# lkotipal/dccrg

Measured on AMD Instinct MI355X. Metric: cell-updates/s (node) for 3D advection w/ halo exchange; % of HBM roofline, higher is better.
Workload: dtype f64

## Files before the change

dccrg_amd/_lib.py:

```python
from __future__ import annotations

import ctypes as C
import os
import re

HERE = os.path.dirname(os.path.abspath(__file__))
LIB_PATH = os.path.join(HERE, os.path.basename(os.environ.get("DCCRGX_LIB", "libdccrgx.so")))
HEADER = os.path.join(os.path.dirname(HERE), "include", "dccrgx.h")

_lib = None

EXCHANGE_FN = C.CFUNCTYPE(C.c_int, C.c_void_p, C.POINTER(C.c_void_p), C.POINTER(C.c_size_t), C.POINTER(C.c_void_p),
                          C.POINTER(C.c_size_t))

u64 = C.c_uint64
i64 = C.c_int64
i32 = C.c_int32
sz = C.c_size_t
vp = C.c_void_p
P = C.POINTER

_SIGS = {
    "dccrgx_last_error": (C.c_char_p, []),
    "dccrgx_abi_version": (C.c_int, []),
# ... 103 lines not shown
    "dccrgx_particles_accelerate": (C.c_int, [vp, C.c_int, C.c_int, C.c_int, C.c_int, C.c_double]),
    "dccrgx_particles_deposit_moments": (C.c_int, [vp, C.c_int, C.c_int, C.c_int, C.c_int, P(C.c_int), P(C.c_int),
                                                   C.c_int, C.c_int]),
    "dccrgx_particles_boris": (C.c_int, [vp, C.c_int, C.c_int, C.c_int, C.c_int, C.c_int, C.c_double]),
    "dccrgx_gradient": (C.c_int, [vp, C.c_int, P(C.c_int), C.c_double, C.c_int]),
    "dccrgx_curl": (C.c_int, [vp, P(C.c_int), P(C.c_int), C.c_double, C.c_int, C.c_int]),
    "dccrgx_divergence": (C.c_int, [vp, P(C.c_int), C.c_int, C.c_double, C.c_int, C.c_int]),
    "dccrgx_field_axpy": (C.c_int, [vp, C.c_int, C.c_double, C.c_int, C.c_int]),
    "dccrgx_set_send_single_cells": (C.c_int, [vp, C.c_int]),
    "dccrgx_get_send_single_cells": (C.c_int, [vp, P(C.c_int)]),
    "dccrgx_set_field_window": (C.c_int, [vp, C.c_int, sz, sz]),
    "dccrgx_field_device_ptr": (C.c_int, [vp, C.c_int, P(vp)]),
    "dccrgx_field_upload": (C.c_int, [vp, C.c_int, sz, sz, vp]),
    "dccrgx_field_download": (C.c_int, [vp, C.c_int, sz, sz, vp]),
    "dccrgx_update_copies_of_remote_neighbors": (C.c_int, [vp]),
    "dccrgx_start_remote_neighbor_copy_updates": (C.c_int, [vp]),
    "dccrgx_wait_remote_neighbor_copy_update_receives": (C.c_int, [vp]),
    "dccrgx_wait_remote_neighbor_copy_update_sends": (C.c_int, [vp]),
    "dccrgx_wait_remote_neighbor_copy_updates": (C.c_int, [vp]),
    "dccrgx_gol_step": (C.c_int, [vp, C.c_int, C.c_int]),
    "dccrgx_gol_commit": (C.c_int, [vp, C.c_int]),
    "dccrgx_gol_amr": (C.c_int, [vp, C.c_int, C.c_int, C.c_int, C.c_int]),
    "dccrgx_get_live_neighbors": (C.c_int, [vp, C.c_int, C.c_int]),
    "dccrgx_advection_step": (C.c_int, [vp, P(C.c_int), C.c_double, C.c_int]),
    "dccrgx_advection_commit": (C.c_int, [vp, C.c_int]),
    "dccrgx_advection_initialize": (C.c_int, [vp, P(C.c_int)]),
    "dccrgx_advection_max_time_step": (C.c_int, [vp, P(C.c_int), P(C.c_double)]),
    "dccrgx_advection_max_time_step_device": (C.c_int, [vp, P(C.c_int), vp]),
    "dccrgx_advection_check_adaptation": (C.c_int, [vp, C.c_int, C.c_double, C.c_double, C.c_double, vp]),
    "dccrgx_advection_adapt": (C.c_int, [vp, vp, vp]),
    "dccrgx_advection_refine_candidates": (C.c_int, [vp, C.c_int, C.c_double, C.c_double, vp, sz, P(sz)]),
    "dccrgx_advection_layout": (C.c_int, [vp, P(u64)]),
    "dccrgx_advection_occupancy": (C.c_int, [vp, P(u64)]),
    "dccrgx_advection_length_source": (C.c_int, [vp, P(C.c_int), P(C.c_int)]),
    "dccrgx_poisson_cache": (C.c_int, [vp, C.c_int, C.c_int, vp, sz, vp, sz]),
    "dccrgx_poisson_solve": (C.c_int, [vp, C.c_uint, C.c_uint, C.c_double, C.c_double, C.c_double, C.c_int,
                                       P(C.c_uint), P(C.c_double)]),
    "dccrgx_poisson_field": (C.c_int, [vp, C.c_char_p, P(C.c_int)]),
    "dccrgx_allreduce_f64": (C.c_int, [vp, P(C.c_double), C.c_int, C.c_int]),
    "dccrgx_allreduce_f64_device": (C.c_int, [vp, vp, vp, C.c_int, C.c_int]),
    "dccrgx_barrier": (C.c_int, [vp]),
    "dccrgx_get_transport": (C.c_int, [vp, P(C.c_int), P(C.c_int)]),
    "dccrgx_comm_loopback": (C.c_int, [vp, C.c_int, sz, sz, sz]),
    "dccrgx_synchronize": (C.c_int, [vp]),
    "dccrgx_compute_stream": (vp, [vp]),
    "dccrgx_kernel_timing": (C.c_int, [vp, C.c_int, P(C.c_double), P(i64)]),
}


def header_symbols():
    with open(HEADER) as f:
        txt = f.read()
    return sorted(set(re.findall(r"\b(dccrgx_[a-z0-9_]+)\s*\(", txt)))


def lib():
    global _lib
    if _lib is not None:
        return _lib
    if not os.path.exists(LIB_PATH):
        raise ImportError(f"dccrg_amd native library missing: {LIB_PATH} (run python -m dccrg_amd.build)")
    L = C.CDLL(LIB_PATH)
    for name, (res, args) in _SIGS.items():
        fn = getattr(L, name)
        fn.restype = res
        fn.argtypes = args
# ... 18 lines not shown
```

dccrg_amd/csrc/api.hip:

```cpp
#include <algorithm>
#include <array>
#include <chrono>
#include <cmath>
#include <cstdio>
#include <cstring>
#include <limits>
#include <numeric>

#include <fcntl.h>
#include <unistd.h>

#include "dccrgx_grid.hpp"

namespace dccrgx {

static thread_local std::string g_last_error;

template <class F>
static int guard(F&& f) {
	try {
		return f();
	} catch (const Error& e) {
		g_last_error = e.what();
		return e.code;
// ... 2639 lines not shown
		const char* env = std::getenv("DCCRGX_NBREC");
		const bool rec_off = !(env && std::atoi(env) == 1);
		uint64_t per_ext = rec_off ? 40 : 32;
		const uint64_t n_irr_cells = n - out[9], ext_irr = g.total_ext - ext_reg;
		uint64_t own = 64, lvl_byte = 0;
		if (g.adv_fids_valid && ensure_len_table(g, g.adv_fids, false)) {
			per_ext = 16;
			lvl_byte = 1;
			if (DCCRGX_LEN_OWN) own = 40;
		}
		out[11] = own * n + (12 + (own == 40 ? lvl_byte : 0)) * n_irr_cells + (per_ext + lvl_byte + 4) * ext_irr +
		          per_ext * ext_reg + 8 * uint64_t(g.n_fine_faces) + 32 * nt;
		return 0;
	});
}

int dccrgx_advection_occupancy(dccrgx_grid* gp, uint64_t out[6]) {
	return guard([&] {
		GRID_OR_FAIL(gp);
		DX_REQUIRE(out, "null output");
		ensure_tiles(g);
		const bool valid = g.adv_fids_valid;
		const bool rec = valid && ensure_nbrec(g, g.adv_fids) != nullptr;
		const bool len = valid && ensure_len_table(g, g.adv_fids, false) != nullptr;
		for (int kind = 0; kind < 2; kind++) {
			const Grid::SweepLaunch& L = adv_sweep_launch(g, kind, rec, len);
			int k = 0;
			HIP_CHECK(hipOccupancyMaxActiveBlocksPerMultiprocessor(&k, L.fn, 512, L.lds));
			out[3 * kind] = uint64_t(L.blocks_per_cu);
			out[3 * kind + 1] = uint64_t(k);
			out[3 * kind + 2] = L.lds;
		}
		return 0;
	});
}

int dccrgx_advection_length_source(dccrgx_grid* gp, const int fids[7], int* out) {
	return guard([&] {
		GRID_OR_FAIL(gp);
		DX_REQUIRE(out, "null output");
		const double* f[7];
		adv_fields(g, fids, f);
		ensure_tiles(g);
		*out = ensure_len_table(g, fids, false) ? 1 : 0;
		return 0;
	});
}

int dccrgx_advection_commit(dccrgx_grid* gp, int df) {
	return guard([&] {
		GRID_OR_FAIL(gp);
		commit(g, field(g, df));
		g.adv_commits_on_mesh++;
		return 0;
	});
}

int dccrgx_advection_initialize(dccrgx_grid* gp, const int fids[7]) {
	return guard([&] {
		GRID_OR_FAIL(gp);
		const auto& ids = slot_ids_host(g);
		const size_t n = g.n_slots;
		for (int k = 0; k < 7; k++) g.adv_fids[k] = fids[k];
		g.adv_fids_valid = true;
		const bool stretched = g.str.active;
		for (int d = 0; d < 3 && stretched; d++)
// ... 544 lines not shown
```

dccrg_amd/csrc/dccrgx_internal.hpp:

```cpp
#pragma once

#include <hip/hip_runtime.h>
#include <rccl/rccl.h>

#include <atomic>
#include <cstdint>
#include <deque>
#include <map>
#include <stdexcept>
#include <string>
#include <unordered_map>
#include <unordered_set>
#include <vector>

#include "../../include/dccrgx.h"
#include "dccrgx_mapping.hpp"
#include "dccrgx_mesh.hpp"
#include "dccrgx_neighbors.hpp"

namespace dccrgx {

struct Error : std::runtime_error {
	int code;
	Error(int c, const std::string& s) : std::runtime_error(s), code(c) {}
// ... 705 lines not shown
                     size_t n_prefix = 0, const DevMesh* dm = nullptr, DBuf<int32_t>* src = nullptr,
                     const uint64_t* dS = nullptr, const uint64_t* dF = nullptr);

struct TileBuild {
	size_t n_tiles_inner = 0, n_tiles_outer = 0, max_ext = 0, total_ext = 0, n_fine = 0;
	std::vector<uint32_t> ext_off, ext_n, fine_off, fine_n;
};
TileBuild k_build_tiles(const uint32_t* face_ptr, const int32_t* face_ent, const uint64_t* slot_ids, const MapCtx& m,
                        bool morton, size_t n_inner, size_t n_local, int tile, DBuf<uint32_t>& tstart,
                        DBuf<uint32_t>& tell, DBuf<uint32_t>& ext_ptr, DBuf<uint32_t>& ext, DBuf<uint32_t>& ext_pk,
                        DBuf<uint32_t>& fine_base, DBuf<uint32_t>& tfine, hipStream_t s);

void k_classify_tiles(const MapCtx& m, const uint32_t* tstart, size_t n_tiles_inner, size_t n_tiles_outer,
                      const uint64_t* slot_ids, const int32_t* face_ell, DBuf<uint32_t>& lists, DBuf<int32_t>& tnb,
                      DBuf<RegTileMeta>& regmeta, size_t counts[4], hipStream_t s);

void k_pack(const uint8_t* field, size_t elem, size_t off, size_t len, const int32_t* slots, size_t n, uint8_t* out,
            hipStream_t s);
void k_place(const uint8_t* in, size_t elem, size_t off, size_t len, const int32_t* slots, size_t n, uint8_t* field,
             hipStream_t s);
void k_gol_csr(const uint32_t* state, uint32_t* out, const uint32_t* it_ptr, const int32_t* it_slot, size_t s0,
               size_t s1, hipStream_t s);
bool k_gol_structured(const uint32_t* state, uint32_t* out, const uint64_t n[3], const int per[3], const uint32_t* lo,
                      const uint32_t* hi, hipStream_t s);
void k_advection(const double* const f[7], double* rho_out, const uint32_t* face_ptr, const int32_t* face_ent,
                 size_t s0, size_t s1, double dt, hipStream_t s);
void k_advection_tiles(const double* const f[7], double* rho_out, Grid& g, int run, double dt, hipStream_t s,
                       const double* nbrec = nullptr, const double* lentab = nullptr);
const double* ensure_len_table(Grid& g, const int fids[7], bool sweep);
void k_len_check(const double* const f[7], const uint8_t* slot_lvl, size_t n, const double* tab, int* flag,
                 hipStream_t s);
void k_tile_levels(const uint8_t* slot_lvl, const uint32_t* ext_pk, size_t n_ext, uint8_t* ext_lvl,
                   RegTileMeta* regmeta, size_t n_reg, hipStream_t s);
#ifndef DCCRGX_LEN_OWN
#define DCCRGX_LEN_OWN 1
#endif
#ifndef DCCRGX_LEN_LDS
#define DCCRGX_LEN_LDS 0
#endif
#ifndef DCCRGX_LEN_LDS_GEN
#define DCCRGX_LEN_LDS_GEN DCCRGX_LEN_LDS
#endif
#ifndef DCCRGX_REG_BLOCKS
#define DCCRGX_REG_BLOCKS ((DCCRGX_LEN_OWN && !DCCRGX_LEN_LDS) ? 3 : 2)
#endif
#ifndef DCCRGX_GEN_BLOCKS
#define DCCRGX_GEN_BLOCKS ((DCCRGX_LEN_OWN && !DCCRGX_LEN_LDS_GEN) ? 3 : 2)
#endif
const Grid::SweepLaunch& adv_sweep_launch(Grid& g, int kind, bool nbrec, bool lentab);
const double* ensure_nbrec(Grid& g, const int fids[7]);
void k_nbrec(const double* const f[7], size_t n, double* r, hipStream_t s);
struct BandArgs {
	MapCtx m;
	const uint8_t* lvl8;
	const uint64_t* slot_ids;
	double inc, thr, uns;
	uint8_t* band;
};
void k_advection_ell(const double* const f[7], double* rho_out, const int32_t* ell, const int32_t* fine, size_t s0,
                     size_t s1, double dt, hipStream_t s, const BandArgs* bands = nullptr);
void k_adv_dt(const double* const f[7], size_t n, double* partial, size_t nblocks, hipStream_t s);
void k_min_partials(const double* partial, size_t n, double* out, hipStream_t s);
size_t k_adv_candidates(const MapCtx& m, const double* rho, const FaceView& F, const uint8_t* lvl8, size_t n,
                        double diff_increase, double diff_threshold, uint64_t* out, hipStream_t s);
struct AdvRequests {
	std::vector<uint64_t> refine, unrefine;
	DBuf<uint64_t> refine_dev;
	DBuf<uint64_t> unrefine_dev;
	size_t kept = 0;
	std::vector<size_t> part_slot;
	std::vector<uint32_t> part_len;
	std::vector<uint64_t> part_ids;
	std::vector<uint8_t> part_bands;
};
AdvRequests k_adv_requests(const MapCtx& m, const DevMesh& dm, const uint64_t* slot_ids, const uint8_t* band, size_t n,
                           bool solo, int rank, hipStream_t s);
void k_adv_bands(const MapCtx& m, const double* rho, const FaceView& F, const uint8_t* lvl8, size_t n,
                 double diff_increase, double diff_threshold, double unrefine_sensitivity, uint8_t* band,
                 hipStream_t s);
void k_adv_merge_parents(const MapCtx& m, const DevMesh& dm, size_t n_local, LazyIds& rm, double* rho,
// ... 65 lines not shown
```

dccrg_amd/csrc/mesh.hip:

```cpp
#include <algorithm>
#include <cstring>
#include <numeric>
#include <set>

#include "dccrgx_grid.hpp"

namespace dccrgx {

namespace {

__global__ void select_owner_kernel(const uint64_t* ids, const int32_t* own, size_t n, int rank, uint64_t* out,
                                    unsigned long long* counter) {
	const size_t i0 = (blockIdx.x * size_t(blockDim.x) + threadIdx.x) * kAppendRun;
	unsigned c = 0;
	for (int k = 0; k < kAppendRun; k++)
		if (i0 + k < n && own[i0 + k] == rank) c++;
	unsigned long long at = wave_reserve(counter, c);
	for (int k = 0; k < kAppendRun && c; k++)
		if (i0 + k < n && own[i0 + k] == rank) {
			out[at++] = ids[i0 + k];
			c--;
		}
}

// ... 688 lines not shown
	const auto ts = download(g.tstart.p, nt + 1, g.s_comp);
	const auto li = download(g.tlists.p + g.tcount[0] + g.tcount[1], ni, g.s_comp);
	std::vector<uint32_t> rec(8 * ni, 0u);
	bool fits = true;
	for (size_t i = 0; i < ni; i++) {
		const uint32_t t = li[i];
		uint32_t* r = &rec[8 * i];
		r[0] = ts[t];
		r[1] = ts[t + 1] - ts[t];
		r[2] = tb.ext_off[t];
		r[3] = tb.ext_n[t];
		r[4] = tb.fine_off[t];
		r[5] = tb.fine_n[t];
		if (r[3] > 1024u || r[5] > 512u || r[1] > 512u) fits = false;
	}
	if (std::getenv("DCCRGX_TILE_REASONS") && ni) {
		std::map<uint32_t, size_t> hist;
		uint32_t emax = 0;
		size_t etot = 0, ax_n[4] = {0, 0, 0, 0};
		const auto pk = download(g.ext_pk.p, g.total_ext, g.s_comp);
		for (size_t i = 0; i < ni; i++) {
			const uint32_t e = rec[8 * i + 3];
			hist[e / 128u * 128u]++;
			emax = std::max(emax, e);
			etot += e;
			for (uint32_t k = 0; k < e; k++) ax_n[__builtin_popcount(pk[rec[8 * i + 2] + k] >> 29)]++;
		}
		std::fprintf(stderr, "[tiles] irregular: %zu tiles, ext total %zu, max %u (all tiles: max %zu)\n", ni, etot, emax,
		             g.max_ext);
		for (auto& kv : hist) std::fprintf(stderr, "[tiles] ext %u..%u: %zu tiles\n", kv.first, kv.first + 127, kv.second);
		std::fprintf(stderr, "[tiles] ext axes per entry: 0:%zu 1:%zu 2:%zu 3:%zu\n", ax_n[0], ax_n[1], ax_n[2], ax_n[3]);
	}
	g.tmeta.release();
	if (fits && ni) upload(g.tmeta, rec, g.s_comp);
	g.tfused.release();
	g.tfused_n[0] = g.tfused_n[1] = 0;
#if DCCRGX_FUSED_SWEEP
	if (fits && nt) {
		const size_t nr = g.tcount[0] + g.tcount[1];
		const auto lr = download(g.tlists.p, nr, g.s_comp);
		std::vector<RegTileMeta> rm(nr);
		if (nr) d2h_small(rm.data(), g.tregmeta.p, nr * sizeof(RegTileMeta), g.s_comp);
		std::vector<int64_t> where(nt, -1);
		for (size_t i = 0; i < nr; i++) where[lr[i]] = int64_t(i);
		for (size_t i = 0; i < ni; i++) where[li[i]] = -int64_t(i) - 2;
		std::vector<uint32_t> fu(8 * nt, 0u);
		for (size_t t = 0; t < nt; t++) {
			uint32_t* r = &fu[8 * t];
			if (where[t] >= 0) {
				const RegTileMeta& m = rm[size_t(where[t])];
				r[0] = m.ts;
				for (int d = 0; d < 6; d++) r[1 + d] = uint32_t(m.nst[d]);
				r[7] = 1u;
			} else {
				const uint32_t* q = &rec[8 * size_t(-where[t] - 2)];
				for (int k = 0; k < 8; k++) r[k] = q[k];
			}
		}
		upload(g.tfused, fu, g.s_comp);
		g.tfused_n[0] = g.n_tiles_inner;
		g.tfused_n[1] = g.n_tiles_outer;
	}
#endif
	HIP_CHECK(hipStreamSynchronize(g.s_comp));
	DX_LAP("tiles.3_meta");
	g.tiles_valid = true;
	g.tiles_gen++;
// ... 80 lines not shown
```

dccrg_amd/csrc/sweep_kernels.hip:

```cpp
#include <cstring>
#include <cstdlib>

#include "dccrgx_internal.hpp"

namespace dccrgx {

namespace {

template <class T>
__global__ void pack_kernel(const T* __restrict__ f, const int32_t* __restrict__ slots, size_t n, T* __restrict__ out) {
	for (size_t i = blockIdx.x * size_t(blockDim.x) + threadIdx.x; i < n; i += size_t(gridDim.x) * blockDim.x)
		out[i] = f[slots[i]];
}

template <class T>
__global__ void place_kernel(const T* __restrict__ in, const int32_t* __restrict__ slots, size_t n, T* __restrict__ f) {
	for (size_t i = blockIdx.x * size_t(blockDim.x) + threadIdx.x; i < n; i += size_t(gridDim.x) * blockDim.x)
		f[slots[i]] = in[i];
}

__global__ void pack_bytes_kernel(const uint8_t* __restrict__ f, size_t elem, size_t off, size_t len,
                                  const int32_t* __restrict__ slots, size_t n, uint8_t* __restrict__ out) {
	for (size_t i = blockIdx.x * size_t(blockDim.x) + threadIdx.x; i < n * len; i += size_t(gridDim.x) * blockDim.x) {
		const size_t k = i / len, b = i - k * len;
// ... 905 lines not shown
	uint32_t tn = tk.next(t);
	uint32_t rec = tn < t1 ? tile_record_word(meta, tn, lane) : 0u;
	for (;;) {
		{
			RegSet ra;
			load(cur, ra);
			__syncthreads();
			stage(ra);
		}
		__syncthreads();
		const bool more = tn < t1;
		RM nxt = cur;
		if (more) {
			nxt = unpack(rec);
			const uint32_t tnn = tk.next(tn);
			rec = tnn < t1 ? tile_record_word(meta, tnn, lane) : 0u;
		}
		compute(cur);
		if (!more) break;
		cur = nxt;
		tn = tk.next(tn);
	}
}

struct TileMeta {
	uint32_t ts, n, e0, ne, fb, nf, pad0, pad1;
};

template <int MINW, bool REC, bool ONCE, bool LEN>
__global__ __launch_bounds__(512, MINW) void advection_tiles_pp_kernel(
    AdvPtrs P, double* __restrict__ rho_out, const uint32_t* __restrict__ tell, uint32_t tplane,
    const uint32_t* __restrict__ ext, const uint32_t* __restrict__ tfine, const TileMeta* __restrict__ meta,
    uint32_t ntiles, uint32_t ecap, double dt, const double* __restrict__ R, size_t nrec,
    const uint8_t* __restrict__ slvl, const uint8_t* __restrict__ extl, const double* __restrict__ LT) {
#pragma clang fp contract(off)
	static_assert(!(LEN && (REC || ONCE)), "the length table is for the default kernels only");
	constexpr bool LOWN = LEN && DCCRGX_LEN_OWN;
	constexpr bool LLVL = LOWN && !DCCRGX_LEN_LDS_GEN;
	constexpr uint32_t T = 512;
	constexpr uint32_t NROW = LLVL ? 4 : 7;
	extern __shared__ double shd[];
	const uint32_t W = T + ecap;
	double* shg = shd + NROW * W;
	uint32_t* shf = reinterpret_cast<uint32_t*>(shd + NROW * W + (ONCE ? 3 * T : 0));
	uint8_t* shok = reinterpret_cast<uint8_t*>(shf + 2 * T);
	double* lt = reinterpret_cast<double*>(shf + 2 * T);
	uint8_t* shl = reinterpret_cast<uint8_t*>(lt + 96);
	const StaticTiles tk(ntiles);
	const uint32_t t1 = tk.t1;
	uint32_t t = tk.first();
	if (t >= t1) return;
	const uint32_t tid = threadIdx.x;
	uint32_t ti = tid;
	const double* const rho = P.p[0];
	const double* const lx = P.p[1];
	const double* const ly = P.p[2];
	const double* const lz = P.p[3];
	const double* const vx = P.p[4];
	const double* const vy = P.p[5];
	const double* const vz = P.p[6];
	double c[7], xa[7], xb[7];
	uint32_t row[3], fq[2];
	uint32_t lvc = 0, lva = 0, lvb = 0;
	if (LEN && tid < 96u) lt[tid] = LT[tid];
	auto load7 = [&](uint32_t slot, double (&v)[7]) {
		const uint32_t o = slot << 3;
		v[0] = ldo(rho, o); v[1] = ldo(vx, o); v[2] = ldo(vy, o); v[3] = ldo(vz, o);
// ... 5 lines not shown
	};
	auto lengths = [&](uint32_t lv, double (&v)[7]) {
		const uint32_t k = 3u * (lv & 31u);
		v[4] = lt[k]; v[5] = lt[k + 1]; v[6] = lt[k + 2];
	};
	auto load5 = [&](uint32_t q, double (&v)[7]) {
		const uint32_t sl = q & 0x1fffffffu, o = sl << 3, ax = q >> 29;
		v[0] = ldo(rho, o);
		if (LEN) {
			v[1] = (ax & 1u) ? ldo(vx, o) : 0.0;
			v[2] = (ax & 2u) ? ldo(vy, o) : 0.0;
			v[3] = (ax & 4u) ? ldo(vz, o) : 0.0;
			return;
		}
		if (REC && (ax == 1u || ax == 2u || ax == 4u)) {
			const uint32_t a = ax >> 1;
			const double* r = R + size_t(a) * 3 * nrec + 3 * size_t(sl);
			const double la = r[0], ar = r[1], vv = r[2];
			v[4] = a == 0 ? la : ar;
			v[5] = a == 0 ? ar : (a == 1 ? la : 1.0);
			v[6] = a == 2 ? la : 1.0;
			v[1] = a == 0 ? vv : 0.0;
			v[2] = a == 1 ? vv : 0.0;
			v[3] = a == 2 ? vv : 0.0;
			return;
		}
		v[4] = ldo(lx, o); v[5] = ldo(ly, o); v[6] = ldo(lz, o);
		v[1] = (ax & 1u) ? ldo(vx, o) : 0.0;
		v[2] = (ax & 2u) ? ldo(vy, o) : 0.0;
		v[3] = (ax & 4u) ? ldo(vz, o) : 0.0;
	};
	const uint32_t lane = tid & 63u;
	struct GM {
		uint32_t ts, n, e0, ne, fb, nf;
	};
	auto unpack = [&](uint32_t v) { return GM{word_of(v, 0), word_of(v, 1), word_of(v, 2), word_of(v, 3), word_of(v, 4),
	                                          word_of(v, 5)}; };
	auto load = [&](const GM& mt) {
		const uint32_t ts = mt.ts, n = mt.n, e0 = mt.e0, ne = mt.ne, fb = mt.fb, nf = mt.nf;
		if (tid < n) {
			load7(ts + ti, c);
			row[0] = __builtin_nontemporal_load(tell + (ts + ti));
			row[1] = __builtin_nontemporal_load(tell + tplane + (ts + ti));
			row[2] = __builtin_nontemporal_load(tell + 2 * tplane + (ts + ti));
		}
		if (tid < ne) {
			load5(__builtin_nontemporal_load(ext + e0 + ti), xa);
			if (LEN) lva = __builtin_nontemporal_load(extl + e0 + ti);
		}
		if (!LLVL && tid + T < ne) {
			load5(__builtin_nontemporal_load(ext + e0 + tid + T), xb);
			if (LEN) lvb = __builtin_nontemporal_load(extl + e0 + tid + T);
		}
		if (tid < nf) {
			typedef unsigned int u2v __attribute__((ext_vector_type(2)));
			const u2v q = __builtin_nontemporal_load(reinterpret_cast<const u2v*>(tfine) + (fb + ti));
			fq[0] = q.x;
			fq[1] = q.y;
		}
	};
	GM cur = unpack(tile_record_word(meta, t, lane));
	uint32_t tn = tk.next(t);
	load(cur);
	uint32_t rec = tn < t1 ? tile_record_word(meta, tn, lane) : 0u;
	for (;;) {
		const uint32_t n = cur.n, ne = cur.ne, nf = cur.nf, ts = cur.ts;
		if (LLVL) asm volatile("" : "+v"(ti));
		__syncthreads();
		if (tid < n) {
			if (LOWN && !LLVL) lengths(lvc, c);
// ... 6 lines not shown
#pragma unroll
			for (uint32_t k = 0; k < NROW; k++) shd[k * W + T + ti] = xa[k];
			if (LLVL) shl[T + ti] = uint8_t(lva);
		}
		if (tid + T < ne) {
			if (LLVL) {
				load5(__builtin_nontemporal_load(ext + cur.e0 + ti + T), xb);
				lvb = __builtin_nontemporal_load(extl + cur.e0 + ti + T);
				shl[2 * T + ti] = uint8_t(lvb);
			} else if (LEN) {
				lengths(lvb, xb);
			}
#pragma unroll
			for (uint32_t k = 0; k < NROW; k++) shd[k * W + 2 * T + ti] = xb[k];
		}
		if (tid < nf) {
			shf[2 * ti] = fq[0];
			shf[2 * ti + 1] = fq[1];
		}
		const uint32_t r0 = row[0], r1 = row[1], r2 = row[2];
		__syncthreads();
		const bool more = tn < t1;
		GM nxt = cur;
		if (more) {
			nxt = unpack(rec);
			load(nxt);
			const uint32_t tnn = tk.next(tn);
			rec = tnn < t1 ? tile_record_word(meta, tnn, lane) : 0u;
		}
		const bool own = tid < n;
		double cd = 0, cvx = 0, cvy = 0, cvz = 0, clx = 1, cly = 1, clz = 1;
		if (own) {
			cd = shd[ti];
			cvx = shd[W + ti];
			cvy = shd[2 * W + ti];
			cvz = shd[3 * W + ti];
			if (LLVL) {
				const uint32_t k = 3u * (uint32_t(shl[ti]) & 31u);
				clx = lt[k]; cly = lt[k + 1]; clz = lt[k + 2];
			} else {
				clx = shd[(4 % NROW) * W + ti];
				cly = shd[(5 % NROW) * W + ti];
				clz = shd[(6 % NROW) * W + ti];
			}
		}
		auto fetch = [&](uint32_t li, int d) -> AdvNb {
			if (LLVL) {
				const uint32_t k = 3u * (uint32_t(shl[li]) & 31u);
				return AdvNb{shd[li], lt[k], lt[k + 1], lt[k + 2], shd[(1 + (d >> 1)) * W + li]};
			}
			return AdvNb{shd[li], shd[(4 % NROW) * W + li], shd[(5 % NROW) * W + li], shd[(6 % NROW) * W + li],
			             shd[(1 + (d >> 1)) * W + li]};
		};
		const uint32_t rr[3] = {r0, r1, r2};
		double gp[3] = {0, 0, 0};
		bool hp[3] = {false, false, false};
		if (ONCE) {
			if (own) {
				const double cva[3] = {cvx, cvy, cvz};
#pragma unroll
				for (int a = 0; a < 3; a++) {
					const uint32_t code = rr[a] >> 16;
					hp[a] = code < n;
					if (hp[a]) {
						gp[a] = adv_face_g(a, cd, clx, cly, clz, cva[a], fetch(code, 2 * a + 1), dt);
						shg[a * T + tid] = gp[a];
					}
					shok[a * T + tid] = hp[a] ? 1 : 0;
				}
			}
			__syncthreads();
		}
		if (own) {
			double acc = 0;
#pragma unroll
			for (int d = 0; d < 6; d++) {
				const uint32_t code = (rr[d >> 1] >> (16 * (d & 1))) & 0xffffu;
				if (code == 0xffffu) continue;
				if (ONCE) {
					const int a = d >> 1;
					if ((d & 1) && hp[a]) {
						acc += -gp[a];
						continue;
					}
					if (!(d & 1) && code < n && shok[a * T + code]) {
						acc += shg[a * T + code];
						continue;
					}
				}
				if (code & 0x8000u) {
					const uint32_t fk = code & 0x7fffu;
					const uint32_t q0 = shf[2 * fk], q1 = shf[2 * fk + 1];
					const uint32_t li[4] = {q0 & 0xffffu, q0 >> 16, q1 & 0xffffu, q1 >> 16};
#pragma unroll
					for (int k = 0; k < 4; k++)
						acc += adv_face_flux_d(d, cd, clx, cly, clz, cvx, cvy, cvz, fetch(li[k], d), dt);
				} else {
					acc += adv_face_flux_d(d, cd, clx, cly, clz, cvx, cvy, cvz, fetch(code, d), dt);
				}
			}
			st_nt(rho_out, ts + ti, cd + acc / (clx * cly * clz));
		}
		if (!more) break;
		cur = nxt;
		tn = tk.next(tn);
	}
// ... 723 lines not shown
		const unsigned nblk = unsigned(std::min<size_t>(size_t(256) * 2, (nt + 7) / 8 * 8));
		advection_fused_kernel<4><<<nblk, 512, std::max(lgen, lreg), s>>>(
		    P, rho_out, g.tell.p, uint32_t(g.n_local + 1), g.ext_pk.p, g.tfine.p, meta, uint32_t(nt), ecap, dt);
		HIP_CHECK(hipGetLastError());
		return;
	}
#endif
	if (n_reg) {
		const RegTileMeta* meta = g.tregmeta.p + (run == 0 ? 0 : g.tcount[0]);
		static const bool reg3 = std::getenv("DCCRGX_REG3") && std::atoi(std::getenv("DCCRGX_REG3")) == 1;
		if (reg3) {
			const unsigned nblk = unsigned(std::min<size_t>(size_t(256) * 3, (n_reg + 7) / 8 * 8));
			advection_regular3_kernel<6><<<nblk, 512, 0, s>>>(P, rho_out, meta, uint32_t(n_reg), dt);
		} else {
			const Grid::SweepLaunch& L = adv_sweep_launch(g, 0, nbrec != nullptr, lentab != nullptr);
			const unsigned nblk = unsigned(std::min<size_t>(size_t(256) * L.blocks_per_cu, (n_reg + 7) / 8 * 8));
			if (nbrec)
				advection_regular_pp_kernel<4, true, false><<<nblk, 512, L.lds, s>>>(P, rho_out, meta, uint32_t(n_reg),
				                                                                     dt, nbrec, g.n_slots, nullptr);
			else if (lentab)
				advection_regular_pp_kernel<kRegWaves, false, true><<<nblk, 512, L.lds, s>>>(
				    P, rho_out, meta, uint32_t(n_reg), dt, nullptr, 0, lentab);
			else
				advection_regular_pp_kernel<4, false, false><<<nblk, 512, L.lds, s>>>(P, rho_out, meta, uint32_t(n_reg),
				                                                                      dt, nullptr, 0, nullptr);
		}
		HIP_CHECK(hipGetLastError());
	}
	if (n_irr) {
		const TileMeta* meta = reinterpret_cast<const TileMeta*>(g.tmeta.p) + (run == 0 ? 0 : g.tcount[2]);
		const uint32_t ecap = uint32_t(g.max_ext);
		const bool once = adv_face_once();
		const bool len = lentab && !nbrec && !once;
		const Grid::SweepLaunch& L = adv_sweep_launch(g, 1, nbrec != nullptr, lentab != nullptr);
		const size_t lds = L.lds;
		const unsigned nblk = unsigned(std::min<size_t>(size_t(256) * L.blocks_per_cu, (n_irr + 7) / 8 * 8));
		const uint32_t tp = uint32_t(g.n_local + 1);
		if (nbrec && once)
			advection_tiles_pp_kernel<4, true, true, false><<<nblk, 512, lds, s>>>(
			    P, rho_out, g.tell.p, tp, g.ext_pk.p, g.tfine.p, meta, uint32_t(n_irr), ecap, dt, nbrec, g.n_slots, nullptr,
			    nullptr, nullptr);
		else if (nbrec)
			advection_tiles_pp_kernel<4, true, false, false><<<nblk, 512, lds, s>>>(
			    P, rho_out, g.tell.p, tp, g.ext_pk.p, g.tfine.p, meta, uint32_t(n_irr), ecap, dt, nbrec, g.n_slots, nullptr,
			    nullptr, nullptr);
		else if (once)
			advection_tiles_pp_kernel<4, false, true, false><<<nblk, 512, lds, s>>>(
			    P, rho_out, g.tell.p, tp, g.ext_pk.p, g.tfine.p, meta, uint32_t(n_irr), ecap, dt, nullptr, 0, nullptr,
			    nullptr, nullptr);
		else if (len)
			advection_tiles_pp_kernel<kGenWaves, false, false, true><<<nblk, 512, lds, s>>>(
			    P, rho_out, g.tell.p, tp, g.ext_pk.p, g.tfine.p, meta, uint32_t(n_irr), ecap, dt, nullptr, 0, g.slot_lvl.p,
			    g.ext_lvl.p, lentab);
		else
			advection_tiles_pp_kernel<4, false, false, false><<<nblk, 512, lds, s>>>(
			    P, rho_out, g.tell.p, tp, g.ext_pk.p, g.tfine.p, meta, uint32_t(n_irr), ecap, dt, nullptr, 0, nullptr,
			    nullptr, nullptr);
		HIP_CHECK(hipGetLastError());
	}
}

__global__ void len_check_kernel(const double* __restrict__ lx, const double* __restrict__ ly,
                                 const double* __restrict__ lz, const uint8_t* __restrict__ lvl, size_t n,
                                 const double* __restrict__ tab, int* __restrict__ flag) {
	bool bad = false;
	for (size_t s = blockIdx.x * size_t(blockDim.x) + threadIdx.x; s < n; s += size_t(gridDim.x) * blockDim.x) {
		const double* r = tab + 3u * (lvl[s] & 31u);
		bad |= __double_as_longlong(lx[s]) != __double_as_longlong(r[0]) ||
		       __double_as_longlong(ly[s]) != __double_as_longlong(r[1]) ||
		       __double_as_longlong(lz[s]) != __double_as_longlong(r[2]);
	}
	if (bad) atomicOr(flag, 1);
}

void k_len_check(const double* const f[7], const uint8_t* slot_lvl, size_t n, const double* tab, int* flag,
                 hipStream_t s) {
	HIP_CHECK(hipMemsetAsync(flag, 0, sizeof(int), s));
	if (!n) return;
	len_check_kernel<<<grid_for(n, 256, 256u * 16u), 256, 0, s>>>(f[4], f[5], f[6], slot_lvl, n, tab, flag);
	HIP_CHECK(hipGetLastError());
}

void k_nbrec(const double* const f[7], size_t n, double* r, hipStream_t s) {
	if (!n) return;
	nbrec_kernel<<<grid_for(n, 256), 256, 0, s>>>(f[4], f[5], f[6], f[1], f[2], f[3], n, r);
	HIP_CHECK(hipGetLastError());
}

void k_adv_dt(const double* const f[7], size_t n, double* partial, size_t nblocks, hipStream_t s) {
	adv_dt_kernel<<<unsigned(nblocks), 256, 0, s>>>(f[1], f[2], f[3], f[4], f[5], f[6], n, partial);
// ... 183 lines not shown
```

dccrg_amd/csrc/tile_build.hip:

```cpp
#include <hipcub/hipcub.hpp>

#include <algorithm>
#include <map>
#include <cstdio>
#include <cstdlib>

#include "dccrgx_internal.hpp"

namespace dccrgx {

namespace {

struct TileGeom {
	const uint32_t* tstart;
	uint32_t ntiles, n_local;
	__device__ void of(uint32_t r, uint32_t& gt, uint32_t& ts, uint32_t& te) const {
		uint32_t lo = 0, hi = ntiles;
		while (hi - lo > 1) {
			const uint32_t mid = (lo + hi) / 2;
			if (tstart[mid] <= r) lo = mid;
			else hi = mid;
		}
		gt = lo;
		ts = tstart[lo];
// ... 785 lines not shown
	h2d(lists.p, all.data(), all.size() * 4, s);
	const std::vector<uint32_t> hts = download(tstart, nt + 1, s);
	const std::vector<int32_t> hnb = download(tnb.p, 6 * nt, s);
	std::vector<RegTileMeta> meta;
	for (int run = 0; run < 2; run++)
		for (uint32_t t : reg[run]) {
			RegTileMeta r{};
			r.ts = hts[t];
			for (int d = 0; d < 6; d++) r.nst[d] = hnb[6 * size_t(t) + d];
			meta.push_back(r);
		}
	regmeta.alloc(meta.size() + 1);
	if (!meta.empty())
		h2d(regmeta.p, meta.data(), meta.size() * sizeof(RegTileMeta), s);
	HIP_CHECK(hipStreamSynchronize(s));
}

__global__ void tile_levels_kernel(const uint8_t* __restrict__ slot_lvl, const uint32_t* __restrict__ ext_pk,
                                   size_t n_ext, uint8_t* __restrict__ ext_lvl, RegTileMeta* __restrict__ regmeta,
                                   size_t n_reg) {
	const size_t stride = size_t(gridDim.x) * blockDim.x, i0 = blockIdx.x * size_t(blockDim.x) + threadIdx.x;
	for (size_t k = i0; k < n_ext; k += stride) ext_lvl[k] = slot_lvl[ext_pk[k] & 0x1fffffffu] & 31u;
	for (size_t k = i0; k < n_reg; k += stride) regmeta[k].pad = slot_lvl[regmeta[k].ts] & 31u;
}

void k_tile_levels(const uint8_t* slot_lvl, const uint32_t* ext_pk, size_t n_ext, uint8_t* ext_lvl,
                   RegTileMeta* regmeta, size_t n_reg, hipStream_t s) {
	const size_t n = std::max(n_ext, n_reg);
	if (!n) return;
	tile_levels_kernel<<<grid_for(n, 256), 256, 0, s>>>(slot_lvl, ext_pk, n_ext, ext_lvl, regmeta, n_reg);
	HIP_CHECK(hipGetLastError());
}

}
```

dccrg_amd/grid.py:

```python
from __future__ import annotations

import ctypes as C
import os

import numpy as np

from ._lib import EINVAL, ENOTFOUND, ERANGE, EXCHANGE_FN, DccrgError, check, lib

REGION = {"all": 0, "inner": 1, "outer": 2}
DEFAULT_HOOD = -0xDCC
CELLS = {"local": 0, "inner": 1, "outer": 2, "remote": 3, "all": 4}
CSR_KIND = {"of": 0, "to": 1, "face": 2, "iterator": 3}
HAS_NO_NEIGHBOR, HAS_LOCAL_NEIGHBOR_OF, HAS_LOCAL_NEIGHBOR_TO = 0, 1, 2
HAS_REMOTE_NEIGHBOR_OF, HAS_REMOTE_NEIGHBOR_TO = 4, 8
HAS_LOCAL_NEIGHBOR_BOTH, HAS_REMOTE_NEIGHBOR_BOTH = 3, 12


def _ptr(a):
    return a.ctypes.data_as(C.c_void_p) if a is not None else None


def _dev_ptr(t):
    if isinstance(t, int):
        return C.c_void_p(t)
# ... 870 lines not shown
        check(lib().dccrgx_advection_initialize(self.h, self._fids(fields)))

    def advection_max_time_step(self, fields):
        v = C.c_double()
        check(lib().dccrgx_advection_max_time_step(self.h, self._fids(fields), C.byref(v)))
        return self.allreduce(v.value, "min")

    def advection_max_time_step_device(self, fields, out):
        check(lib().dccrgx_advection_max_time_step_device(self.h, self._fids(fields), _dev_ptr(out)))

    def advection_length_source(self, fields):
        v = C.c_int()
        check(lib().dccrgx_advection_length_source(self.h, self._fids(fields), C.byref(v)))
        return v.value

    def advection_layout(self):
        out = (C.c_uint64 * 12)()
        check(lib().dccrgx_advection_layout(self.h, out))
        keys = ("tile", "tiles", "ext_total", "ext_max", "finer_faces", "face_entries", "alg_bytes",
                "alg_bytes_core", "regular_tiles", "regular_cells", "ext_regular", "bytes_needed")
        lay = dict(zip(keys, (int(v) for v in out)))
        occ = self.advection_occupancy()
        lay["regular_blocks_per_cu"] = occ["regular"]["blocks_per_cu"]
        lay["general_blocks_per_cu"] = occ["general"]["blocks_per_cu"]
        return lay

    def advection_occupancy(self):
        out = (C.c_uint64 * 6)()
        check(lib().dccrgx_advection_occupancy(self.h, out))
        v = [int(x) for x in out]
        keys = ("blocks_per_cu", "blocks_per_cu_query", "lds_bytes")
        return {"regular": dict(zip(keys, v[0:3])), "general": dict(zip(keys, v[3:6]))}

    def advection_check_adaptation(self, density, diff_increase, diff_threshold=0.25, unrefine_sensitivity=0.5):
        c = np.zeros(3, np.uint64)
        check(lib().dccrgx_advection_check_adaptation(self.h, density.id, float(diff_increase), float(diff_threshold),
                                                      float(unrefine_sensitivity), _ptr(c)))
        return tuple(int(x) for x in c)

    def advection_adapt(self, fields):
        out = np.zeros(2, np.uint64)
        check(lib().dccrgx_advection_adapt(self.h, self._fids(fields), _ptr(out)))
        return int(out[0]), int(out[1])

    def advection_refine_candidates(self, density, diff_increase, diff_threshold):
        return self._u64_query(lib().dccrgx_advection_refine_candidates, density.id, float(diff_increase),
                               float(diff_threshold))

    def allreduce(self, value, op="sum"):
        v = C.c_double(float(value))
        check(lib().dccrgx_allreduce_f64(self.h, C.byref(v), 1, {"sum": 0, "min": 1, "max": 2}[op]))
        return v.value

    def allreduce_device(self, src, dst=None, op="sum"):
        n = int(src.numel()) if hasattr(src, "numel") else None
        if n is None:
            raise TypeError("allreduce_device needs a torch tensor (its element count)")
        d = src if dst is None else dst
        check(lib().dccrgx_allreduce_f64_device(self.h, _dev_ptr(src), _dev_ptr(d), n,
                                                {"sum": 0, "min": 1, "max": 2}[op]))

    def transport(self):
        k, n = C.c_int(), C.c_int()
        check(lib().dccrgx_get_transport(self.h, C.byref(k), C.byref(n)))
        return ("none", "rccl", "host")[k.value], n.value

# ... 11 lines not shown
```

include/dccrgx.h:

```cpp
#ifndef DCCRGX_H
#define DCCRGX_H

#include <stddef.h>
#include <stdint.h>

#ifdef __cplusplus
extern "C" {
#endif

typedef struct dccrgx_grid dccrgx_grid;

#define DCCRGX_ABI_VERSION 10

#define DCCRGX_OK 0
#define DCCRGX_EINVAL -1
#define DCCRGX_EHIP -2
#define DCCRGX_ECOMM -3
#define DCCRGX_ERANGE -4
#define DCCRGX_ENOTFOUND -5

#define DCCRGX_CELLS_LOCAL 0
#define DCCRGX_CELLS_INNER 1
#define DCCRGX_CELLS_OUTER 2
#define DCCRGX_CELLS_REMOTE 3
// ... 154 lines not shown

int dccrgx_set_send_single_cells(dccrgx_grid* g, int on);
int dccrgx_get_send_single_cells(dccrgx_grid* g, int* on);

int dccrgx_update_copies_of_remote_neighbors(dccrgx_grid* g);
int dccrgx_start_remote_neighbor_copy_updates(dccrgx_grid* g);
int dccrgx_wait_remote_neighbor_copy_update_receives(dccrgx_grid* g);
int dccrgx_wait_remote_neighbor_copy_update_sends(dccrgx_grid* g);
int dccrgx_wait_remote_neighbor_copy_updates(dccrgx_grid* g);
int dccrgx_halo_message_size(dccrgx_grid* g, int hood_id, int peer, size_t* send_bytes, size_t* recv_bytes);
int dccrgx_halo_pack(dccrgx_grid* g, int hood_id, int peer, void* buf, size_t cap);
int dccrgx_halo_place(dccrgx_grid* g, int hood_id, int peer, const void* buf, size_t bytes);

int dccrgx_gol_step(dccrgx_grid* g, int state_field, int region);
int dccrgx_gol_commit(dccrgx_grid* g, int state_field);

int dccrgx_gol_amr(dccrgx_grid* g, int phase, int state_field, int list_field, int region);
int dccrgx_get_live_neighbors(dccrgx_grid* g, int state_field, int list_field);
int dccrgx_advection_step(dccrgx_grid* g, const int fields[7], double dt, int region);
int dccrgx_advection_commit(dccrgx_grid* g, int density_field);
int dccrgx_advection_initialize(dccrgx_grid* g, const int fields[7]);
int dccrgx_advection_max_time_step(dccrgx_grid* g, const int fields[7], double* local_min);
int dccrgx_advection_max_time_step_device(dccrgx_grid* g, const int fields[7], double* d_out);
int dccrgx_advection_refine_candidates(dccrgx_grid* g, int density_field, double diff_increase,
                                       double diff_threshold, uint64_t* out, size_t cap, size_t* n);

int dccrgx_advection_check_adaptation(dccrgx_grid* g, int density_field, double diff_increase,
                                      double diff_threshold, double unrefine_sensitivity, uint64_t counts[3]);
int dccrgx_advection_adapt(dccrgx_grid* g, const int fields[7], uint64_t out[2]);
int dccrgx_advection_layout(dccrgx_grid* g, uint64_t out[12]);

int dccrgx_advection_occupancy(dccrgx_grid* g, uint64_t out[6]);

int dccrgx_advection_length_source(dccrgx_grid* g, const int fids[7], int* out);

int dccrgx_poisson_cache(dccrgx_grid* g, int rhs_field, int solution_field, const uint64_t* solve_cells,
                         size_t n_solve, const uint64_t* skip_cells, size_t n_skip);
int dccrgx_poisson_solve(dccrgx_grid* g, unsigned max_iterations, unsigned min_iterations, double stop_residual,
                         double p_of_norm, double stop_after_residual_increase, int failsafe, unsigned* iterations,
                         double* residual);
int dccrgx_poisson_field(dccrgx_grid* g, const char* name, int* field_id);

int dccrgx_allreduce_f64(dccrgx_grid* g, double* inout, int count, int op );
int dccrgx_allreduce_f64_device(dccrgx_grid* g, const double* d_in, double* d_out, int count, int op);
int dccrgx_barrier(dccrgx_grid* g);

#define DCCRGX_TRANSPORT_NONE 0
#define DCCRGX_TRANSPORT_RCCL 1
#define DCCRGX_TRANSPORT_HOST 2
int dccrgx_get_transport(dccrgx_grid* g, int* kind, int* comm_ranks);

int dccrgx_comm_loopback(dccrgx_grid* g, int field_id, size_t slot0, size_t n, size_t dst_slot0);

int dccrgx_synchronize(dccrgx_grid* g);
void* dccrgx_compute_stream(dccrgx_grid* g);
int dccrgx_kernel_timing(dccrgx_grid* g, int enable, double* total_ms, int64_t* count);

#ifdef __cplusplus
}
#endif

#endif
```

Baseline: 71.49 billion.

## Add per-wave plain-level fast path in irregular advection tile kernel

At tile build time, a new kernel marks which 64-lane waves of each irregular tile have every neighbor at the same refinement level, and stores this as a bitmask in a spare tile-metadata word. The length-table sweep kernel reads that mask and, for plain waves, runs a simplified per-axis flux loop that loads velocities lazily and assumes equal lengths. Other waves keep the general path. This aims to cut per-face level and length work and register pressure on mostly uniform tiles, at the cost of an extra metadata kernel, a divergent code path and a larger kernel. It also adds a debug query API that exposes the masks.

Result: no change. 71.97 billion, median of 3 (+0.7%).

```diff
diff --git a/dccrg_amd/_lib.py b/dccrg_amd/_lib.py
--- a/dccrg_amd/_lib.py
+++ b/dccrg_amd/_lib.py
@@ -159,6 +159,7 @@
     "dccrgx_advection_refine_candidates": (C.c_int, [vp, C.c_int, C.c_double, C.c_double, vp, sz, P(sz)]),
     "dccrgx_advection_layout": (C.c_int, [vp, P(u64)]),
     "dccrgx_advection_occupancy": (C.c_int, [vp, P(u64)]),
+    "dccrgx_advection_tile_waves": (C.c_int, [vp, vp, sz, P(sz)]),
     "dccrgx_advection_length_source": (C.c_int, [vp, P(C.c_int), P(C.c_int)]),
     "dccrgx_poisson_cache": (C.c_int, [vp, C.c_int, C.c_int, vp, sz, vp, sz]),
     "dccrgx_poisson_solve": (C.c_int, [vp, C.c_uint, C.c_uint, C.c_double, C.c_double, C.c_double, C.c_int,
diff --git a/dccrg_amd/csrc/api.hip b/dccrg_amd/csrc/api.hip
--- a/dccrg_amd/csrc/api.hip
+++ b/dccrg_amd/csrc/api.hip
@@ -2695,6 +2695,22 @@
 			out[3 * kind + 2] = L.lds;
 		}
 		return 0;
+	});
+}
+
+int dccrgx_advection_tile_waves(dccrgx_grid* gp, uint64_t* out, size_t cap, size_t* n) {
+	return guard([&] {
+		GRID_OR_FAIL(gp);
+		ensure_tiles(g);
+		const size_t ni = g.tmeta.n ? g.tcount[2] + g.tcount[3] : 0;
+		const std::vector<uint32_t> rec = download(g.tmeta.p, 8 * ni, g.s_comp);
+		std::vector<uint64_t> v(3 * ni);
+		for (size_t i = 0; i < ni; i++) {
+			v[3 * i] = rec[8 * i];
+			v[3 * i + 1] = rec[8 * i + 1];
+			v[3 * i + 2] = rec[8 * i + 6];
+		}
+		return copy_out_u64(v, out, cap, n);
 	});
 }
 
diff --git a/dccrg_amd/csrc/dccrgx_internal.hpp b/dccrg_amd/csrc/dccrgx_internal.hpp
--- a/dccrg_amd/csrc/dccrgx_internal.hpp
+++ b/dccrg_amd/csrc/dccrgx_internal.hpp
@@ -761,6 +761,8 @@
                  hipStream_t s);
 void k_tile_levels(const uint8_t* slot_lvl, const uint32_t* ext_pk, size_t n_ext, uint8_t* ext_lvl,
                    RegTileMeta* regmeta, size_t n_reg, hipStream_t s);
+void k_tile_plain_waves(uint32_t* meta, size_t n_tiles, uint32_t T, const uint32_t* tell, size_t pl,
+                        const uint8_t* slot_lvl, const uint8_t* ext_lvl, hipStream_t s);
 #ifndef DCCRGX_LEN_OWN
 #define DCCRGX_LEN_OWN 1
 #endif
@@ -775,6 +777,9 @@
 #endif
 #ifndef DCCRGX_GEN_BLOCKS
 #define DCCRGX_GEN_BLOCKS ((DCCRGX_LEN_OWN && !DCCRGX_LEN_LDS_GEN) ? 3 : 2)
+#endif
+#ifndef DCCRGX_PLAIN_AXES
+#define DCCRGX_PLAIN_AXES 1
 #endif
 const Grid::SweepLaunch& adv_sweep_launch(Grid& g, int kind, bool nbrec, bool lentab);
 const double* ensure_nbrec(Grid& g, const int fids[7]);
diff --git a/dccrg_amd/csrc/mesh.hip b/dccrg_amd/csrc/mesh.hip
--- a/dccrg_amd/csrc/mesh.hip
+++ b/dccrg_amd/csrc/mesh.hip
@@ -744,7 +744,10 @@
 		std::fprintf(stderr, "[tiles] ext axes per entry: 0:%zu 1:%zu 2:%zu 3:%zu\n", ax_n[0], ax_n[1], ax_n[2], ax_n[3]);
 	}
 	g.tmeta.release();
-	if (fits && ni) upload(g.tmeta, rec, g.s_comp);
+	if (fits && ni) {
+		upload(g.tmeta, rec, g.s_comp);
+		k_tile_plain_waves(g.tmeta.p, ni, uint32_t(T), g.tell.p, g.n_local + 1, g.slot_lvl.p, g.ext_lvl.p, g.s_comp);
+	}
 	g.tfused.release();
 	g.tfused_n[0] = g.tfused_n[1] = 0;
 #if DCCRGX_FUSED_SWEEP
diff --git a/dccrg_amd/csrc/sweep_kernels.hip b/dccrg_amd/csrc/sweep_kernels.hip
--- a/dccrg_amd/csrc/sweep_kernels.hip
+++ b/dccrg_amd/csrc/sweep_kernels.hip
@@ -961,7 +961,8 @@
     AdvPtrs P, double* __restrict__ rho_out, const uint32_t* __restrict__ tell, uint32_t tplane,
     const uint32_t* __restrict__ ext, const uint32_t* __restrict__ tfine, const TileMeta* __restrict__ meta,
     uint32_t ntiles, uint32_t ecap, double dt, const double* __restrict__ R, size_t nrec,
-    const uint8_t* __restrict__ slvl, const uint8_t* __restrict__ extl, const double* __restrict__ LT) {
+    const uint8_t* __restrict__ slvl, const uint8_t* __restrict__ extl, const double* __restrict__ LT,
+    uint32_t wmask) {
 #pragma clang fp contract(off)
 	static_assert(!(LEN && (REC || ONCE)), "the length table is for the default kernels only");
 	constexpr bool LOWN = LEN && DCCRGX_LEN_OWN;
@@ -1033,10 +1034,11 @@
 	};
 	const uint32_t lane = tid & 63u;
 	struct GM {
-		uint32_t ts, n, e0, ne, fb, nf;
+		uint32_t ts, n, e0, ne, fb, nf, pw;
 	};
 	auto unpack = [&](uint32_t v) { return GM{word_of(v, 0), word_of(v, 1), word_of(v, 2), word_of(v, 3), word_of(v, 4),
-	                                          word_of(v, 5)}; };
+	                                          word_of(v, 5), LLVL ? word_of(v, 6) & wmask : 0u}; };
+	const uint32_t wave = __builtin_amdgcn_readfirstlane(tid >> 6);
 	auto load = [&](const GM& mt) {
 		const uint32_t ts = mt.ts, n = mt.n, e0 = mt.e0, ne = mt.ne, fb = mt.fb, nf = mt.nf;
 		if (tid < n) {
@@ -1109,9 +1111,11 @@
 		double cd = 0, cvx = 0, cvy = 0, cvz = 0, clx = 1, cly = 1, clz = 1;
 		if (own) {
 			cd = shd[ti];
-			cvx = shd[W + ti];
-			cvy = shd[2 * W + ti];
-			cvz = shd[3 * W + ti];
+			if (!LLVL) {
+				cvx = shd[W + ti];
+				cvy = shd[2 * W + ti];
+				cvz = shd[3 * W + ti];
+			}
 			if (LLVL) {
 				const uint32_t k = 3u * (uint32_t(shl[ti]) & 31u);
 				clx = lt[k]; cly = lt[k + 1]; clz = lt[k + 2];
@@ -1148,7 +1152,41 @@
 			}
 			__syncthreads();
 		}
-		if (own) {
+		if (LLVL && ((cur.pw >> wave) & 1u)) {
+			if (own) {
+				double acc = 0;
+				constexpr int NA = DCCRGX_PLAIN_AXES;
+#pragma unroll
+				for (int a0 = 0; a0 < 3; a0 += NA) {
+					double cva[NA], nd[2 * NA], nv[2 * NA];
+					bool has[2 * NA];
+#pragma unroll
+					for (int j = 0; j < 2 * NA; j++) {
+						const int d = 2 * a0 + j;
+						const uint32_t code = (rr[d >> 1] >> (16 * (d & 1))) & 0xffffu;
+						has[j] = code != 0xffffu;
+						const uint32_t li = has[j] ? code : ti;
+						if (!(j & 1)) cva[j >> 1] = shd[(1 + (d >> 1)) * W + ti];
+						nd[j] = shd[li];
+						nv[j] = shd[(1 + (d >> 1)) * W + li];
+					}
+#pragma unroll
+					for (int j = 0; j < 2 * NA; j++) {
+						const int d = 2 * a0 + j;
+						const double cv = cva[j >> 1];
+						const double fl = adv_face_flux_d(d, cd, clx, cly, clz, cv, cv, cv, AdvNb{nd[j], clx, cly, clz, nv[j]}, dt);
+						acc += has[j] ? fl : 0.0;
+					}
+					__builtin_amdgcn_sched_barrier(0);
+				}
+				st_nt(rho_out, ts + ti, cd + acc / (clx * cly * clz));
+			}
+		} else if (own) {
+			if (LLVL) {
+				cvx = shd[W + ti];
+				cvy = shd[2 * W + ti];
+				cvz = shd[3 * W + ti];
+			}
 			double acc = 0;
 #pragma unroll
 			for (int d = 0; d < 6; d++) {
@@ -1938,6 +1976,8 @@
 		const uint32_t ecap = uint32_t(g.max_ext);
 		const bool once = adv_face_once();
 		const bool len = lentab && !nbrec && !once;
+		const char* pwv = std::getenv("DCCRGX_PLAIN_WAVES");
+		const bool plain = !(pwv && pwv[0] == '0');
 		const Grid::SweepLaunch& L = adv_sweep_launch(g, 1, nbrec != nullptr, lentab != nullptr);
 		const size_t lds = L.lds;
 		const unsigned nblk = unsigned(std::min<size_t>(size_t(256) * L.blocks_per_cu, (n_irr + 7) / 8 * 8));
@@ -1945,23 +1985,23 @@
 		if (nbrec && once)
 			advection_tiles_pp_kernel<4, true, true, false><<<nblk, 512, lds, s>>>(
 			    P, rho_out, g.tell.p, tp, g.ext_pk.p, g.tfine.p, meta, uint32_t(n_irr), ecap, dt, nbrec, g.n_slots, nullptr,
-			    nullptr, nullptr);
+			    nullptr, nullptr, 0u);
 		else if (nbrec)
 			advection_tiles_pp_kernel<4, true, false, false><<<nblk, 512, lds, s>>>(
 			    P, rho_out, g.tell.p, tp, g.ext_pk.p, g.tfine.p, meta, uint32_t(n_irr), ecap, dt, nbrec, g.n_slots, nullptr,
-			    nullptr, nullptr);
+			    nullptr, nullptr, 0u);
 		else if (once)
 			advection_tiles_pp_kernel<4, false, true, false><<<nblk, 512, lds, s>>>(
 			    P, rho_out, g.tell.p, tp, g.ext_pk.p, g.tfine.p, meta, uint32_t(n_irr), ecap, dt, nullptr, 0, nullptr,
-			    nullptr, nullptr);
+			    nullptr, nullptr, 0u);
 		else if (len)
 			advection_tiles_pp_kernel<kGenWaves, false, false, true><<<nblk, 512, lds, s>>>(
 			    P, rho_out, g.tell.p, tp, g.ext_pk.p, g.tfine.p, meta, uint32_t(n_irr), ecap, dt, nullptr, 0, g.slot_lvl.p,
-			    g.ext_lvl.p, lentab);
+			    g.ext_lvl.p, lentab, plain ? 0xffu : 0u);
 		else
 			advection_tiles_pp_kernel<4, false, false, false><<<nblk, 512, lds, s>>>(
 			    P, rho_out, g.tell.p, tp, g.ext_pk.p, g.tfine.p, meta, uint32_t(n_irr), ecap, dt, nullptr, 0, nullptr,
-			    nullptr, nullptr);
+			    nullptr, nullptr, 0u);
 		HIP_CHECK(hipGetLastError());
 	}
 }
diff --git a/dccrg_amd/csrc/tile_build.hip b/dccrg_amd/csrc/tile_build.hip
--- a/dccrg_amd/csrc/tile_build.hip
+++ b/dccrg_amd/csrc/tile_build.hip
@@ -841,4 +841,42 @@
 	HIP_CHECK(hipGetLastError());
 }
 
-}
+__global__ __launch_bounds__(512) void tile_plain_waves_kernel(uint32_t* __restrict__ meta, uint32_t T,
+                                                               const uint32_t* __restrict__ tell, size_t pl,
+                                                               const uint8_t* __restrict__ slot_lvl,
+                                                               const uint8_t* __restrict__ ext_lvl) {
+	__shared__ uint32_t mask;
+	uint32_t* r = meta + 8 * size_t(blockIdx.x);
+	const uint32_t ts = r[0], n = r[1], e0 = r[2], ne = r[3];
+	const uint32_t tid = threadIdx.x;
+	if (tid == 0) mask = 0;
+	__syncthreads();
+	bool ok = true;
+	if (tid < n) {
+		const uint32_t lv = slot_lvl[ts + tid] & 31u;
+		for (int a = 0; a < 3; a++) {
+			const uint32_t w = tell[size_t(a) * pl + ts + tid];
+			for (int h = 0; h < 2; h++) {
+				const uint32_t code = (w >> (16 * h)) & 0xffffu;
+				if (code == 0xffffu) continue;
+				if (code < n) ok = ok && (slot_lvl[ts + code] & 31u) == lv;
+				else if (code >= T && code - T < ne) ok = ok && (ext_lvl[e0 + (code - T)] & 31u) == lv;
+				else ok = false;
+			}
+		}
+	}
+	const bool all = __all(ok);
+	if ((tid & 63u) == 0 && tid < n && all) atomicOr(&mask, 1u << (tid >> 6));
+	__syncthreads();
+	if (tid == 0) r[6] = mask;
+}
+
+void k_tile_plain_waves(uint32_t* meta, size_t n_tiles, uint32_t T, const uint32_t* tell, size_t pl,
+                        const uint8_t* slot_lvl, const uint8_t* ext_lvl, hipStream_t s) {
+	if (!n_tiles) return;
+	DX_REQUIRE(T == 512, "the plain-wave mask is for tiles of 512 slots");
+	tile_plain_waves_kernel<<<unsigned(n_tiles), 512, 0, s>>>(meta, T, tell, pl, slot_lvl, ext_lvl);
+	HIP_CHECK(hipGetLastError());
+}
+
+}
diff --git a/dccrg_amd/grid.py b/dccrg_amd/grid.py
--- a/dccrg_amd/grid.py
+++ b/dccrg_amd/grid.py
@@ -926,6 +926,9 @@
         keys = ("blocks_per_cu", "blocks_per_cu_query", "lds_bytes")
         return {"regular": dict(zip(keys, v[0:3])), "general": dict(zip(keys, v[3:6]))}
 
+    def advection_tile_waves(self):
+        return self._u64_query(lib().dccrgx_advection_tile_waves).reshape(-1, 3)
+
     def advection_check_adaptation(self, density, diff_increase, diff_threshold=0.25, unrefine_sensitivity=0.5):
         c = np.zeros(3, np.uint64)
         check(lib().dccrgx_advection_check_adaptation(self.h, density.id, float(diff_increase), float(diff_threshold),
diff --git a/include/dccrgx.h b/include/dccrgx.h
--- a/include/dccrgx.h
+++ b/include/dccrgx.h
@@ -210,6 +210,8 @@
 
 int dccrgx_advection_occupancy(dccrgx_grid* g, uint64_t out[6]);
 
+int dccrgx_advection_tile_waves(dccrgx_grid* g, uint64_t* out, size_t cap, size_t* n);
+
 int dccrgx_advection_length_source(dccrgx_grid* g, const int fids[7], int* out);
 
 int dccrgx_poisson_cache(dccrgx_grid* g, int rhs_field, int solution_field, const uint64_t* solve_cells,
```
